# volume-em/empanada

Measured on AMD Instinct MI355X. Metric: Mvox/s end-to-end 3D panoptic inference (incl. consensus); PQ vs CPU ref, higher is better.
Workload: dtype f32

## Files before the change

empanada_amd/_hip.py:

```python
import ctypes
import os

import torch

from .tables import bits

_HERE = os.path.dirname(os.path.abspath(__file__))
LIB_PATH = os.path.join(_HERE, 'libemp_hip.so')

MAX_KS = 11
MAX_CLASSES = 16
MAX_CENTERS = 4096
CENTER_LIMIT = 65535


class HipError(RuntimeError):
    pass


_c = ctypes
_P = _c.c_void_p
_I = _c.c_int
_L = _c.c_int64
_F = _c.c_float
_U32 = _c.c_uint32

SIGNATURES = {
    'emp_version': (_I, []),
    'emp_last_error': (_c.c_char_p, []),
    'emp_device_count': (_I, []),
    'emp_bn_act_nhwc': (_I, [_P, _P, _P, _P, _I, _L, _I, _P, _L, _P]),
    'emp_dwconv_nhwc': (_I, [_P, _P, _P, _I, _I, _I, _I, _I, _P, _P]),
    'emp_upsample_bilinear': (_I, [_P, _I, _I, _I, _I, _P, _P, _I, _I, _P, _P]),
    'emp_conv_bn_act_proj_nhwc': (_I, [_P, _P, _P, _P, _I] + [_I] * 10 + [_P, _I, _P, _P, _L, _P]),
    'emp_conv_k_slab': (_I, [_L, _I, _I, _I]),
    'emp_conv_stream_eligible': (_I, [_I, _L] + [_I] * 9),
    'emp_conv_stream_walk': (_I, [_L, _I, _I, _I, _L, _P, _P]),
    'emp_conv_stream_grid': (_I, [_L, _I]),
    'emp_conv_stream_launches': (_L, []),
    'emp_conv_k_slab_cin': (_I, [_L, _I, _I, _I, _I]),
    'emp_conv_k_slab_geom': (_I, [_L, _I, _I, _I, _I, _I, _I, _I, _I]),
    'emp_conv1x1_ws_eligible': (_I, [_L, _I, _I, _I, _I, _I, _I, _I]),
    'emp_conv1x1_ws_kind_for': (_I, [_L, _I, _I, _I, _I, _I, _I, _I, _I]),
    'emp_conv1x1_ws_launches': (_L, [_I]),
    'emp_gconv_chunk': (_I, [_I]),
    'emp_gconv3x3_bn_act_nhwc': (_I, [_P, _L, _P, _P, _P, _I, _I, _I, _I, _I, _I, _I, _P, _L, _P]),
    'emp_conv_bn_act_nhwc': (_I, [_P, _P, _P, _P, _P, _L, _I] + [_I] * 10 + [_P, _L, _P]),
    'emp_conv_splitk_plan': (_I, [_L, _I, _I, _I, _I]),
    'emp_conv_splitk_bn_act_nhwc': (_I, [_P, _P, _P, _P, _P, _L, _I] + [_I] * 11 + [_P, _P, _L, _P]),
    'emp_wino_input_transform': (_I, [_P, _I, _I, _I, _I, _I, _P, _L, _P, _P]),
    'emp_gemm_nt_batched': (_I, [_P, _P, _I, _L, _I, _I, _P, _P]),
    'emp_wino4_input_transform': (_I, [_P, _I, _I, _I, _I, _I, _P, _L, _P, _P]),
    'emp_wino4_output_transform': (_I, [_P, _P, _L, _I, _I, _I, _I, _I, _P, _P, _I, _P, _L, _P]),
    'emp_wino4_conv_bn_act_nhwc': (_I, [_P, _I, _I, _I, _I, _I, _P, _L, _P, _I, _P, _P, _I, _P, _L, _P]),
    'emp_wino4_fused_eligible': (_I, [_L, _I, _I, _I]),
    'emp_wino3_input_transform': (_I, [_P, _I, _I, _I, _I, _I, _P, _L, _P, _P]),
    'emp_wino3_output_transform': (_I, [_P, _P, _L, _I, _I, _I, _I, _I, _P, _P, _I, _P, _L, _P]),
    'emp_wino_gemm_fused': (_I, [_P, _I, _I, _I, _I, _I, _P, _L, _P, _I, _P, _P]),
    'emp_wino_output_transform': (_I, [_P, _P, _L, _I, _I, _I, _I, _I, _P, _P, _I, _P, _L, _P]),
    'emp_chain_class': (_I, [_L, _P, _P, _P, _I, _P, _P, _P, _P, _L, _L, _c.c_double, _c.c_double, _P, _P, _P, _P]),
    'emp_lsap_maximize': (_L, [_P, _L, _L, _P, _P]),
    'emp_slices_to_input': (_I, [_P, _L, _L, _L, _I, _I, _I, _I, _I, _F, _F, _P, _P]),
    'emp_slices_to_input_scaled': (_I, [_P, _L, _L, _L] + [_I] * 7 + [_P, _P, _P, _P, _I, _F, _F, _P, _P]),
    'emp_pointwise_out_nhwc': (_I, [_P, _P, _P, _L, _L, _I, _I, _P, _P]),
    'emp_bn_relu_maxpool_nhwc': (_I, [_P, _P, _P, _I, _I, _I, _I, _P, _P]),
    'emp_stem_conv7_bn_relu_maxpool': (_I, [_P, _P, _P, _P, _I, _I, _I, _P, _P]),
    'emp_logits_to_prob': (_I, [_P, _I, _I, _L, _P, _P]),
    'emp_upsample_bilinear_prob': (_I, [_P, _I, _I, _I, _I, _P, _P, _I, _I, _P, _I, _P]),
    'emp_pr_upsample2x': (_I, [_P, _I, _I, _I, _I, _P, _P, _P]),
    'emp_pr_topk_work_bytes': (_L, [_I, _L]),
    'emp_pr_topk': (_I, [_P, _I, _L, _I, _P, _L, _P, _P]),
    'emp_pr_point_sample': (_I, [_P, _L, _P, _I, _I, _I, _I, _I, _P, _I, _I, _I, _P, _P, _I, _P]),
    'emp_pr_scatter': (_I, [_P, _I, _P, _I, _I, _I, _L, _P, _P]),
    'emp_median_harden_stack': (_I, [_P, _I, _I, _L, _I, _F, _P, _P, _P]),
    'emp_median_harden_window': (_I, [_P, _P, _P, _I, _I, _L, _I, _F, _P, _P, _P]),
    'emp_median_step': (_I, [_c.POINTER(_P), _I, _L, _P, _P]),
    'emp_harden': (_I, [_P, _I, _I, _L, _F, _P, _P]),
    'emp_find_centers': (_I, [_P, _I, _I, _I, _F, _I, _I, _P, _P, _P]),
    'emp_find_centers_work_elems': (_L, [_I, _I, _I, _I]),
    'emp_find_centers_ws': (_I, [_P, _I, _I, _I, _F, _I, _I, _P, _P, _P, _P]),
    'emp_group_work_elems': (_L, [_I, _I]),
    'emp_group_pixels': (_I, [_P, _P, _I, _P, _I, _I, _I, _I, _P, _U32, _P, _P, _P]),
    'emp_fuse_work_elems': (_L, [_I, _I, _I]),
    'emp_fuse_panoptic': (_I, [_P, _P, _I, _I, _I, _I, _I, _I, _U32, _L, _L, _L, _P, _P, _P, _P]),
    'emp_fuse_lut': (_I, [_P, _P, _I, _I, _I, _I, _I, _I, _U32, _L, _L, _P, _P]),
    'emp_fuse_apply': (_I, [_P, _P, _I, _I, _I, _I, _I, _I, _U32, _L, _L, _P, _P, _P, _P]),
    'emp_runs_count': (_I, [_P, _I, _I, _I, _P, _P]),
# ... 2451 lines not shown
                                               int(stride), int(pad), 2 if relu == 'gate' else int(bool(relu))))
    if Cin is not None:
        return int(load().emp_conv_k_slab_cin(int(M), int(Cout), int(batch), int(bool(has_residual)), int(Cin)))
    return int(load().emp_conv_k_slab(int(M), int(Cout), int(batch), int(bool(has_residual))))


_WINO3_G = [[0.5, 0.0, 0.0], [-0.5, -0.5, -0.5], [-1.0 / 6, 1.0 / 6, -1.0 / 6], [1.0 / 6, 1.0 / 3, 2.0 / 3], [0.0, 0.0, 1.0]]


def wino3_filter_transform(w_oihw):
    g = w_oihw.detach().double().cpu()

    def comb(a, b, c):
        return [(G[0] * a + G[1] * b) + G[2] * c for G in _WINO3_G]

    rows = comb(g[:, :, 0, :], g[:, :, 1, :], g[:, :, 2, :])
    U = []
    for r in rows:
        U.extend(comb(r[:, :, 0], r[:, :, 1], r[:, :, 2]))
    return torch.stack(U, dim=0).float().contiguous()


def wino3_conv_bn_act(x, U, tiles_dev, dil, scale=None, shift=None, relu=False, out=None):
    require_gpu()
    N, Cin, H, W = x.shape
    Cout = U.shape[1]
    assert x.is_cuda and x.dtype == torch.float32 and x.is_contiguous(memory_format=torch.channels_last)
    T = tiles_dev.shape[0]
    V = torch.empty((25, T, Cin), dtype=torch.float32, device=x.device)
    Mw = torch.empty((25, T, Cout), dtype=torch.float32, device=x.device)
    if out is None:
        out = torch.empty((N, Cout, H, W), dtype=torch.float32, device=x.device, memory_format=torch.channels_last)
    assert out.shape == (N, Cout, H, W) and out.stride(1) == 1
    ops = out.stride(3)
    assert out.stride(2) == W * ops and out.stride(0) == H * W * ops, "NHWC channel slice required"
    st = stream()
    call('emp_wino3_input_transform', x.data_ptr(), N, H, W, Cin, dil, _ptr(tiles_dev), T, _ptr(V), st,
         alg_bytes=4 * (x.numel() + V.numel()))
    call('emp_gemm_nt_batched', _ptr(V), _ptr(U), 25, T, Cout, Cin, _ptr(Mw), st,
         alg_bytes=4 * (V.numel() + U.numel() + Mw.numel()), alg_flops=2 * 25 * T * Cout * Cin)
    call('emp_wino3_output_transform', _ptr(Mw), _ptr(tiles_dev), T, N, H, W, Cout, dil, _ptr(scale), _ptr(shift),
         int(bool(relu)), out.data_ptr(), ops, st, alg_bytes=4 * (Mw.numel() + N * Cout * H * W))
    return out


def conv_bn_act_proj_nhwc(x, w_okkc, scale, shift, relu, proj_w, proj_b=None, stride=1, pad=0, dil=1, keep=False):
    require_gpu()
    N, Cin, H, W = x.shape
    Cout, KH, KW, _ = w_okkc.shape
    n = proj_w.shape[0]
    assert x.is_cuda and x.dtype == torch.float32 and x.is_contiguous(memory_format=torch.channels_last)
    OH = (H + 2 * pad - dil * (KH - 1) - 1) // stride + 1
    OW = (W + 2 * pad - dil * (KW - 1) - 1) // stride + 1
    acc = torch.zeros((N, n, OH, OW), dtype=torch.float32, device=x.device)
    act = (torch.empty((N, Cout, OH, OW), dtype=torch.float32, device=x.device, memory_format=torch.channels_last)
           if keep else None)
    call('emp_conv_bn_act_proj_nhwc', x.data_ptr(), _ptr(w_okkc), _ptr(scale), _ptr(shift), int(bool(relu)), N, H, W,
         Cin, Cout, KH, KW, stride, pad, dil, _ptr(proj_w), n, _ptr(acc), act.data_ptr() if keep else None, 0,
         stream(), alg_bytes=4 * (x.numel() + w_okkc.numel() + acc.numel() + (act.numel() if keep else 0)),
         alg_flops=2 * N * OH * OW * Cout * (Cin * KH * KW + n))
    if proj_b is not None:
        acc += proj_b.view(1, -1, 1, 1)
    return (acc, act) if keep else acc
```

empanada_amd/csrc/emp_conv.hip:

```cpp
#include "emp_common.h"
#include "emp_wino4.h"
#include <stdlib.h>

typedef float f32x16 __attribute__((ext_vector_type(16)));

#define CG_BM 128
#define CG_BK 32
#define CG_THREADS 256

struct ConvGeom {
    const float *x, *w, *scale, *shift, *res;
    float *out;
    int N, H, W, Cin, OH, OW, Cout, KH, KW, stride, pad, dil, relu;
    int64_t M, out_ps, res_ps;
    int tiles_m, tiles_n;
    int64_t x_bs, w_bs, out_bs;
    const int32_t *tiles;
    const float *proj_w;
    float *proj_out;
    int proj_n;
    int64_t hw;
};

__device__ __attribute__((aligned(16))) float cg_zero_page[64];
// ... 692 lines not shown
    const int T = g.tiles_m * g.tiles_n;
    const dim3 grid(8 * ((T + 7) / 8), 1, k_splits);
    hipStream_t st = emp_stream(stream);
    if (pl.narrow)
        hipLaunchKernelGGL((conv_igemm_f32_kernel<1, 0, false, 32, false, true>), grid, dim3(CG_THREADS), 0, st, g);
    else
        hipLaunchKernelGGL((conv_igemm_f32_kernel<2, 0, false, 32, false, true>), grid, dim3(CG_THREADS), 0, st, g);
    EMP_CHECK_LAUNCH("emp_conv_splitk_bn_act_nhwc(partials)");
    const int64_t total = g.M * (Cout / 4);
    hipLaunchKernelGGL(splitk_reduce_kernel, dim3(emp_grid(total, 256, 4096)), dim3(256), 0, st, work, k_splits, g.M, Cout,
                       scale, shift, residual, res_pixel_stride, relu, out, out_pixel_stride);
    EMP_CHECK_LAUNCH("emp_conv_splitk_bn_act_nhwc(reduce)");
    return EMP_OK;
}

extern "C" int emp_conv_bn_act_proj_nhwc(const float *x, const float *w_okkc, const float *scale, const float *shift,
                                         int relu, int N, int H, int W, int Cin, int Cout, int KH, int KW, int stride,
                                         int pad, int dil, const float *proj_w, int proj_n, float *proj_out,
                                         float *out, int64_t out_pixel_stride, void *stream)
{
    EMP_REQUIRE(x && w_okkc && proj_w && proj_out, "conv_proj: null pointer");
    EMP_REQUIRE(N >= 0 && H > 0 && W > 0 && Cin > 0 && Cin % CG_BK == 0, "conv_proj: bad shape (Cin %% %d)", CG_BK);
    EMP_REQUIRE(Cout == 128 || Cout == 256, "conv_proj: Cout %d must be 128 or 256 (at most two cout tiles)", Cout);
    EMP_REQUIRE(proj_n >= 1 && proj_n <= 4, "conv_proj: proj_n %d not in 1..4", proj_n);
    EMP_REQUIRE(KH >= 1 && KW >= 1 && KH <= 7 && KW <= 7 && stride >= 1 && dil >= 1 && pad >= 0, "conv_proj: bad filter geometry");
    const int OH = (H + 2 * pad - dil * (KH - 1) - 1) / stride + 1;
    const int OW = (W + 2 * pad - dil * (KW - 1) - 1) / stride + 1;
    EMP_REQUIRE(OH > 0 && OW > 0, "conv_proj: empty output");
    if (out_pixel_stride == 0) out_pixel_stride = Cout;
    EMP_REQUIRE(((reinterpret_cast<uintptr_t>(x) | reinterpret_cast<uintptr_t>(w_okkc) | reinterpret_cast<uintptr_t>(proj_w) |
                  reinterpret_cast<uintptr_t>(out)) & 15) == 0 && (out_pixel_stride & 3) == 0, "conv_proj: alignment");
    EMP_REQUIRE(out != x, "conv_proj: output cannot alias the input");
    if (N == 0) return EMP_OK;
    ConvGeom g;
    g.x = x; g.w = w_okkc; g.scale = scale; g.shift = shift; g.res = nullptr; g.out = out;
    g.N = N; g.H = H; g.W = W; g.Cin = Cin; g.OH = OH; g.OW = OW; g.Cout = Cout; g.KH = KH; g.KW = KW;
    g.stride = stride; g.pad = pad; g.dil = dil; g.relu = relu;
    g.M = (int64_t)N * OH * OW; g.out_ps = out_pixel_stride; g.res_ps = Cout;
    g.x_bs = g.w_bs = g.out_bs = 0; g.tiles = nullptr;
    g.proj_w = proj_w; g.proj_out = proj_out; g.proj_n = proj_n; g.hw = (int64_t)OH * OW;
    const CgPlan pl = cg_plan(g.M, Cout, 1, false, true, false);
    g.tiles_m = pl.tiles_m;
    g.tiles_n = pl.tiles_n;
    const int T = g.tiles_m * g.tiles_n;
    const int grid = 8 * ((T + 7) / 8);
#define CG_GOP(BK_, GL_) hipLaunchKernelGGL((conv_igemm_f32_kernel<2, 0, false, BK_, true, GL_>), dim3(grid), dim3(CG_THREADS), 0, emp_stream(stream), g)
    if (pl.glds) { if (pl.slab == 16) CG_GOP(16, true); else CG_GOP(32, true); }
    else { if (pl.slab == 16) CG_GOP(16, false); else CG_GOP(32, false); }
#undef CG_GOP
    EMP_CHECK_LAUNCH("emp_conv_bn_act_proj_nhwc");
    return EMP_OK;
}


__global__ __launch_bounds__(256) void wino_input_kernel(const float *__restrict__ x, const int32_t *__restrict__ tiles,
                                                         int64_t T, int H, int W, int C4, int dil, float4 *__restrict__ V)
{
    const int64_t total = T * C4;
    for (int64_t i = (int64_t)blockIdx.x * blockDim.x + threadIdx.x; i < total; i += (int64_t)gridDim.x * blockDim.x) {
        const int c4 = (int)(i % C4);
        const int64_t t = i / C4;
        const int n = tiles[3 * t], by = tiles[3 * t + 1], bx = tiles[3 * t + 2];
        const float4 *src = reinterpret_cast<const float4 *>(x) + (int64_t)n * H * W * C4 + c4;
        float4 d[4][4];
#pragma unroll
        for (int a = 0; a < 4; ++a)
#pragma unroll
            for (int b = 0; b < 4; ++b) {
                const int yy = by + a * dil, xx = bx + b * dil;
                d[a][b] = make_float4(0.f, 0.f, 0.f, 0.f);
                if (yy >= 0 && yy < H && xx >= 0 && xx < W) d[a][b] = src[((int64_t)yy * W + xx) * C4];
            }
#define W_SUB(p, q) make_float4(__fsub_rn(p.x, q.x), __fsub_rn(p.y, q.y), __fsub_rn(p.z, q.z), __fsub_rn(p.w, q.w))
#define W_ADD(p, q) make_float4(__fadd_rn(p.x, q.x), __fadd_rn(p.y, q.y), __fadd_rn(p.z, q.z), __fadd_rn(p.w, q.w))
        float4 tt[4][4];
#pragma unroll
        for (int a = 0; a < 4; ++a) {
            tt[a][0] = W_SUB(d[a][0], d[a][2]);
            tt[a][1] = W_ADD(d[a][1], d[a][2]);
            tt[a][2] = W_SUB(d[a][2], d[a][1]);
            tt[a][3] = W_SUB(d[a][1], d[a][3]);
        }
        float4 *dst = V + t * C4 + c4;
        const int64_t ps = T * C4;
#pragma unroll
        for (int v = 0; v < 4; ++v) {
            dst[(0 * 4 + v) * ps] = W_SUB(tt[0][v], tt[2][v]);
            dst[(1 * 4 + v) * ps] = W_ADD(tt[1][v], tt[2][v]);
            dst[(2 * 4 + v) * ps] = W_SUB(tt[2][v], tt[1][v]);
            dst[(3 * 4 + v) * ps] = W_SUB(tt[1][v], tt[3][v]);
        }
    }
}

__global__ __launch_bounds__(256) void wino_output_kernel(const float4 *__restrict__ Mw, const int32_t *__restrict__ tiles,
                                                          int64_t T, int H, int W, int Co4, int dil,
                                                          const float4 *__restrict__ scale, const float4 *__restrict__ shift,
                                                          int relu, float *__restrict__ out, int64_t out_ps)
{
    const int64_t total = T * Co4;
    for (int64_t i = (int64_t)blockIdx.x * blockDim.x + threadIdx.x; i < total; i += (int64_t)gridDim.x * blockDim.x) {
        const int c4 = (int)(i % Co4);
        const int64_t t = i / Co4;
        const int n = tiles[3 * t], oy = tiles[3 * t + 1] + dil, ox = tiles[3 * t + 2] + dil;
        const float4 *src = Mw + t * Co4 + c4;
        const int64_t ps = T * Co4;
// ... 387 lines not shown
```

empanada_amd/csrc/emp_conv_stream.hip:

```cpp
#include "emp_common.h"
#include <atomic>
#include <stdlib.h>
#include <type_traits>

typedef float f32x16 __attribute__((ext_vector_type(16)));

#define CS_BM 128
#define CS_BN 128
#define CS_BK 16
#define CS_THREADS 256
#define CS_RING 3
#define CS_RESIDENT 768

struct StreamGeom {
    const float *x, *w, *scale, *shift;
    float *out;
    int Cin, Cout, tiles_n;
    int64_t M, out_ps;
    int64_t tiles, total;
    int64_t x_bs, w_bs, out_bs;
};

__host__ __device__ static inline int64_t cs_walk(int64_t total, int grid, int b, int64_t step)
{
    const int64_t chunk = (total + 7) >> 3;
    const int64_t local = (b >> 3) + step * (grid >> 3);
    if (local >= chunk) return -1;
    const int64_t u = (b & 7) * chunk + local;
    return u < total ? u : -1;
}
__host__ __device__ static inline int64_t cs_walk_steps(int64_t total, int grid, int b)
{
    const int64_t chunk = (total + 7) >> 3;
    int64_t end = total - (b & 7) * chunk;
    if (end > chunk) end = chunk;
    const int64_t first = b >> 3, stride = grid >> 3;
    return end > first ? (end - first + stride - 1) / stride : 0;
}

extern "C" int emp_conv_stream_walk(int64_t tiles, int batch, int grid, int block, int64_t step, int64_t *entry, int64_t *tile)
{
    if (tiles <= 0 || batch <= 0 || grid <= 0 || (grid & 7) || block < 0 || block >= grid || step < 0) return 0;
    const int64_t u = cs_walk(tiles * batch, grid, block, step);
    if (u < 0 || step >= cs_walk_steps(tiles * batch, grid, block)) return 0;
    if (entry) *entry = u / tiles;
    if (tile) *tile = u % tiles;
    return 1;
}

static inline int cs_grid(int64_t total)
{
    const int64_t g = 8 * ((total + 7) / 8);
    return (int)(g < CS_RESIDENT ? g : CS_RESIDENT);
}
extern "C" int emp_conv_stream_grid(int64_t tiles, int batch) { return tiles > 0 && batch > 0 ? cs_grid(tiles * batch) : 0; }

__device__ __forceinline__ void cs_glds16(const float *base, unsigned lane_off, unsigned lds_byte_addr)
{
    asm volatile("s_mov_b32 m0, %2\n\ts_nop 4\n\tglobal_load_lds_dwordx4 %0, %1" ::"v"(lane_off), "s"(base), "s"(lds_byte_addr) : "memory", "m0");
}
__device__ __forceinline__ void cs_store2(float *dst, float v0, float v1)
{
    asm volatile("global_store_dword %0, %1, off\n\tglobal_store_dword %0, %2, off offset:128" ::"v"(dst), "v"(v0), "v"(v1) : "memory");
}
template <int N>
__device__ __forceinline__ void cs_wait_vm()
{
    asm volatile("s_waitcnt vmcnt(%0)" ::"n"(N) : "memory");
}

template <bool AFFINE, bool RELU>
__global__ __launch_bounds__(CS_THREADS, 3) void conv_stream_f32_kernel(StreamGeom g)
{
    constexpr int BK = CS_BK, TPR = BK / 4, RPP = CS_THREADS / TPR, AR = CS_BM / RPP, BROWS = CS_BN / RPP;
    constexpr int NF4 = BK / 8, RPW = 64 / TPR, NL = AR + BROWS;
    constexpr int A_ELEMS = CS_RING * CS_BM * BK, B_ELEMS = CS_RING * CS_BN * BK;
    __shared__ __attribute__((aligned(16))) float smem[A_ELEMS + B_ELEMS];
    float *As = smem, *Bs = smem + A_ELEMS;

    const int b = blockIdx.x, grid = gridDim.x;
    const int nt = (int)cs_walk_steps(g.total, grid, b);
    if (nt == 0) return;
    const int S = g.Cin / BK;
    const int n_slabs = nt * S;
    const int64_t u0 = cs_walk(g.total, grid, b, 0);
    const int64_t ustep = grid >> 3;

    const int tid = threadIdx.x;
    const int lrow = tid / TPR;
    const int wave = tid >> 6, lane = tid & 63;
    const int wm = wave >> 1, wn = wave & 1;
    const int r = lane & 31, hh = lane >> 5;
    const int csw = (((tid % TPR) ^ ((lrow >> 2) & 3)) * 4);
    const int swz_rd = (r >> 2) & 3;

    auto locate = [&](int64_t u, int64_t &entry, int64_t &m0, int &n0) {
        const unsigned uu = (unsigned)u, tiles = (unsigned)g.tiles, tn_ = (unsigned)g.tiles_n;
        const unsigned e = g.total == g.tiles ? 0u : uu / tiles;
        const unsigned t = uu - e * tiles;
        const unsigned tm = t / tn_;
        entry = e;
        m0 = (int64_t)tm * CS_BM;
        n0 = (int)(t - tm * tn_) * CS_BN;
    };

    const float *a_base = nullptr, *b_base = nullptr;
    unsigned voff_a[AR];
    const unsigned voff_b = (unsigned)(lrow * g.Cin + csw) * 4u;
    int ld_k = 0, ld_c0 = 0, ld_ring = 0;
    auto set_ld_tile = [&](int k) {
        int64_t entry, m0;
        int n0;
        locate(u0 + k * ustep, entry, m0, n0);
        a_base = g.x + entry * g.x_bs + m0 * g.Cin;
        b_base = g.w + entry * g.w_bs + (int64_t)n0 * g.Cin;
        const int last = (int)(g.M - m0 < CS_BM ? g.M - m0 : CS_BM) - 1;
#pragma unroll
        for (int i = 0; i < AR; ++i) {
            const int row = lrow + RPP * i;
            voff_a[i] = (unsigned)((row < last ? row : last) * g.Cin + csw) * 4u;
        }
    };
    const unsigned lds0 = (unsigned)(size_t)(__attribute__((address_space(3))) float *)smem;
    const unsigned a_dst = __builtin_amdgcn_readfirstlane(lds0 + (unsigned)(RPW * wave * BK * 4));
    const unsigned b_dst = __builtin_amdgcn_readfirstlane(lds0 + (unsigned)((A_ELEMS + RPW * wave * BK) * 4));
    auto issue_slab = [&]() {
#pragma unroll
        for (int i = 0; i < AR; ++i)
            cs_glds16(a_base + ld_c0, voff_a[i], a_dst + (unsigned)((ld_ring * CS_BM + RPP * i) * BK * 4));
#pragma unroll
        for (int i = 0; i < BROWS; ++i)
            cs_glds16(b_base + (int64_t)(RPP * i) * g.Cin + ld_c0, voff_b, b_dst + (unsigned)((ld_ring * CS_BN + RPP * i) * BK * 4));
        ld_ring = ld_ring == CS_RING - 1 ? 0 : ld_ring + 1;
        ld_c0 += BK;
        if (ld_c0 == g.Cin) {
            ld_c0 = 0;
            ++ld_k;
            if (ld_k < nt) set_ld_tile(ld_k);
        }
    };

    int cp_k = 0, cp_s = 0, rd_ring = 0;
    int sc_n0 = -1;
    float sc[2] = {1.f, 1.f}, sh[2] = {0.f, 0.f};
    auto load_affine = [&](int n0) {
        if constexpr (AFFINE) {
#pragma unroll
            for (int j = 0; j < 2; ++j) {
                sc[j] = g.scale[n0 + wn * 64 + j * 32 + r];
                sh[j] = g.shift[n0 + wn * 64 + j * 32 + r];
            }
            asm volatile("" : "+v"(sc[0]), "+v"(sc[1]), "+v"(sh[0]), "+v"(sh[1]));
        }
        sc_n0 = n0;
    };

    f32x16 acc[2][2];
#pragma unroll
    for (int i = 0; i < 2; ++i)
#pragma unroll
        for (int j = 0; j < 2; ++j)
#pragma unroll
            for (int q = 0; q < 16; ++q) acc[i][j][q] = 0.f;

    auto epilogue = [&](int k) {
        int64_t entry, m0;
        int n0;
        locate(u0 + k * ustep, entry, m0, n0);
        if (n0 != sc_n0) load_affine(n0);
        float *obase = g.out + entry * g.out_bs + (m0 + wm * 64 + 4 * hh) * g.out_ps + n0 + wn * 64 + r;
        const bool whole = m0 + CS_BM <= g.M;
        auto rows = [&](auto checked) {
#pragma unroll
            for (int i = 0; i < 2; ++i)
#pragma unroll
                for (int q = 0; q < 16; ++q) {
                    const int row = i * 32 + (q & 3) + 8 * (q >> 2);
                    float v[2];
#pragma unroll
                    for (int j = 0; j < 2; ++j) {
                        v[j] = acc[i][j][q];
                        if constexpr (AFFINE) v[j] = __fadd_rn(__fmul_rn(v[j], sc[j]), sh[j]);
                        if constexpr (RELU) v[j] = fmaxf(v[j], 0.f);
                    }
                    if (!decltype(checked)::value || m0 + wm * 64 + 4 * hh + row < g.M) cs_store2(obase + row * g.out_ps, v[0], v[1]);
                }
        };
        if (whole) rows(std::false_type{}); else rows(std::true_type{});
#pragma unroll
        for (int i = 0; i < 2; ++i)
#pragma unroll
            for (int j = 0; j < 2; ++j)
#pragma unroll
                for (int q = 0; q < 16; ++q) acc[i][j][q] = 0.f;
    };

    {
        int64_t entry, m0;
        int n0;
        locate(u0, entry, m0, n0);
        load_affine(n0);
    }
    set_ld_tile(0);

    issue_slab();
    if (n_slabs > 1) issue_slab();
    if (n_slabs > 1) cs_wait_vm<NL>(); else cs_wait_vm<0>();
    __builtin_amdgcn_s_barrier();
    for (int s = 0; s < n_slabs; ++s) {
        const bool more = s + 2 < n_slabs;
        if (more) issue_slab();
        const float *Ar = &As[rd_ring * CS_BM * BK + (wm * 64 + r) * BK];
        const float *Br = &Bs[rd_ring * CS_BN * BK + (wn * 64 + r) * BK];
#pragma unroll
        for (int f = 0; f < NF4; ++f) {
            const int pc = (((hh * NF4 + f) ^ swz_rd) * 4);
            float4 fa[2], fb[2];
#pragma unroll
            for (int i = 0; i < 2; ++i) fa[i] = *reinterpret_cast<const float4 *>(Ar + i * 32 * BK + pc);
#pragma unroll
            for (int j = 0; j < 2; ++j) fb[j] = *reinterpret_cast<const float4 *>(Br + j * 32 * BK + pc);
#pragma unroll
            for (int e = 0; e < 4; ++e) {
                float av[2], bv[2];
#pragma unroll
                for (int i = 0; i < 2; ++i) av[i] = e == 0 ? fa[i].x : e == 1 ? fa[i].y : e == 2 ? fa[i].z : fa[i].w;
#pragma unroll
                for (int j = 0; j < 2; ++j) bv[j] = e == 0 ? fb[j].x : e == 1 ? fb[j].y : e == 2 ? fb[j].z : fb[j].w;
#pragma unroll
                for (int i = 0; i < 2; ++i)
#pragma unroll
                    for (int j = 0; j < 2; ++j)
                        acc[i][j] = __builtin_amdgcn_mfma_f32_32x32x2f32(av[i], bv[j], acc[i][j], 0, 0, 0);
            }
        }
        rd_ring = rd_ring == CS_RING - 1 ? 0 : rd_ring + 1;
        if (more) cs_wait_vm<NL>(); else cs_wait_vm<0>();
        __builtin_amdgcn_s_barrier();
        if (++cp_s == S) {
            epilogue(cp_k);
            cp_s = 0;
            ++cp_k;
        }
    }
}

static std::atomic<int64_t> cs_launches;
extern "C" int64_t emp_conv_stream_launches(void) { return cs_launches.load(); }

extern "C" __attribute__((visibility("hidden"))) int emp_conv_stream_launch(const float *x, const float *w, const float *scale, const float *shift,
                                                                            int relu, int batch, int64_t M, int Cin, int Cout,
                                                                            int64_t x_bs, int64_t w_bs, int64_t out_bs, float *out,
                                                                            int64_t out_ps, void *stream)
{
    EMP_REQUIRE(x && w && out && (scale != nullptr) == (shift != nullptr), "conv_stream: null pointer");
    EMP_REQUIRE(batch >= 1 && M > 0 && Cin > 0 && Cin % CS_BK == 0 && Cout > 0 && Cout % CS_BN == 0, "conv_stream: bad shape");
    EMP_REQUIRE(scale || !relu, "conv_stream: ReLU needs scale and shift");
    StreamGeom g;
    g.x = x; g.w = w; g.scale = scale; g.shift = shift; g.out = out;
    g.Cin = Cin; g.Cout = Cout; g.tiles_n = Cout / CS_BN;
    g.M = M; g.out_ps = out_ps;
    g.tiles = emp_cdiv(M, CS_BM) * g.tiles_n;
    g.total = g.tiles * batch;
    g.x_bs = x_bs; g.w_bs = w_bs; g.out_bs = out_bs;
    const int grid = cs_grid(g.total);
    EMP_REQUIRE(g.total < (1LL << 28) && (g.total / grid + 2) * (Cin / CS_BK) < (1LL << 30), "conv_stream: too many tiles");
    hipStream_t st = emp_stream(stream);
    if (!scale) hipLaunchKernelGGL((conv_stream_f32_kernel<false, false>), dim3(grid), dim3(CS_THREADS), 0, st, g);
    else if (relu) hipLaunchKernelGGL((conv_stream_f32_kernel<true, true>), dim3(grid), dim3(CS_THREADS), 0, st, g);
    else hipLaunchKernelGGL((conv_stream_f32_kernel<true, false>), dim3(grid), dim3(CS_THREADS), 0, st, g);
    EMP_CHECK_LAUNCH("emp_conv_stream_launch");
    ++cs_launches;
    return EMP_OK;
}
```

include/emp_hip.h:

```cpp
#ifndef EMP_HIP_H
#define EMP_HIP_H

#include <stdint.h>

#ifdef __cplusplus
extern "C" {
#endif

#define EMP_OK 0
#define EMP_EINVAL (-1)
#define EMP_ELAUNCH (-2)
#define EMP_ENODEV (-3)

#define EMP_MAX_KS 11
#define EMP_MAX_CLASSES 16
#define EMP_MAX_CENTERS 4096
#define EMP_CENTER_LIMIT 65535

int emp_version(void);
const char *emp_last_error(void);
int emp_device_count(void);

int emp_slices_to_input(const uint8_t *vol, int64_t stride_slice, int64_t stride_row, int64_t stride_col,
                        int n_slices, int h, int w, int hp, int wp, float mean255, float inv_std255,
                        float *out, void *stream);

int emp_slices_to_input_scaled(const uint8_t *vol, int64_t stride_slice, int64_t stride_row, int64_t stride_col,
                               int n_slices, int h, int w, int dh, int dw, int hp, int wp, const int32_t *row_off,
                               const int16_t *row_coef, const int32_t *col_off, const int16_t *col_coef, int area,
                               float mean255, float inv_std255, float *out, void *stream);

int emp_bn_act_nhwc(const float *x, const float *scale, const float *shift, const float *residual,
                    int relu, int64_t n_pixels, int C, float *out, int64_t out_pixel_stride, void *stream);

int emp_dwconv_nhwc(const float *x, const float *w_kkc, const float *bias, int N, int H, int W, int C,
                    int k, float *y, void *stream);

int emp_upsample_bilinear(const float *x, int N, int C, int h, int w, const int64_t *x_strides,
                          float *y, int H, int W, const int64_t *y_strides, void *stream);

int emp_conv_k_slab(int64_t M, int Cout, int batch, int has_residual);
int emp_conv_k_slab_cin(int64_t M, int Cout, int batch, int has_residual, int Cin);
int emp_conv_k_slab_geom(int64_t M, int Cout, int has_residual, int Cin, int KH, int KW, int stride, int pad, int relu);
int emp_conv1x1_ws_eligible(int64_t M, int Cin, int Cout, int KH, int KW, int stride, int pad, int relu);
int emp_conv1x1_ws_kind_for(int64_t M, int Cin, int Cout, int KH, int KW, int stride, int pad, int relu, int has_residual);
int64_t emp_conv1x1_ws_launches(int kind);
int emp_conv_stream_eligible(int batch, int64_t M, int Cin, int Cout, int KH, int KW, int stride, int pad, int relu,
                             int has_residual, int proj);
int emp_conv_stream_grid(int64_t tiles, int batch);
int emp_conv_stream_walk(int64_t tiles, int batch, int grid, int block, int64_t step, int64_t *entry, int64_t *tile);
int64_t emp_conv_stream_launches(void);
int emp_conv_bn_act_nhwc(const float *x, const float *w_okkc, const float *scale, const float *shift,
                         const float *residual, int64_t res_pixel_stride, int relu, int N, int H, int W,
                         int Cin, int Cout, int KH, int KW, int stride, int pad, int dil, float *out,
                         int64_t out_pixel_stride, void *stream);
int emp_conv_splitk_plan(int64_t M, int Cout, int Cin, int KH, int KW);
int emp_conv_splitk_bn_act_nhwc(const float *x, const float *w_okkc, const float *scale, const float *shift,
                                const float *residual, int64_t res_pixel_stride, int relu, int N, int H, int W,
                                int Cin, int Cout, int KH, int KW, int stride, int pad, int dil, int k_splits,
                                float *work, float *out, int64_t out_pixel_stride, void *stream);

int emp_conv_bn_act_proj_nhwc(const float *x, const float *w_okkc, const float *scale, const float *shift,
                              int relu, int N, int H, int W, int Cin, int Cout, int KH, int KW, int stride,
                              int pad, int dil, const float *proj_w, int proj_n, float *proj_out,
                              float *out, int64_t out_pixel_stride, void *stream);

int emp_gconv_chunk(int group_w);
int emp_gconv3x3_bn_act_nhwc(const float *x, int64_t x_pixel_stride, const float *w_okkc, const float *scale,
                             const float *shift, int relu, int N, int H, int W, int groups, int group_w,
                             int stride, float *out, int64_t out_pixel_stride, void *stream);

int emp_wino_input_transform(const float *x, int N, int H, int W, int C, int dil, const int32_t *tiles,
                             int64_t T, float *V, void *stream);
int emp_gemm_nt_batched(const float *A, const float *B, int batch, int64_t M, int N, int K, float *C,
                        void *stream);
int emp_wino_gemm_fused(const float *x, int N, int H, int W, int Cin, int dil, const int32_t *tiles,
                        int64_t T, const float *U, int Cout, float *Mw, void *stream);
int emp_wino_output_transform(const float *Mw, const int32_t *tiles, int64_t T, int N, int H, int W,
                              int Cout, int dil, const float *scale, const float *shift, int relu,
                              float *out, int64_t out_pixel_stride, void *stream);

int emp_wino4_input_transform(const float *x, int N, int H, int W, int C, int dil, const int32_t *tiles,
                              int64_t T, float *V, void *stream);
int emp_wino4_output_transform(const float *Mw, const int32_t *tiles, int64_t T, int N, int H, int W,
                               int Cout, int dil, const float *scale, const float *shift, int relu,
                               float *out, int64_t out_pixel_stride, void *stream);
int emp_wino4_conv_bn_act_nhwc(const float *x, int N, int H, int W, int Cin, int dil, const int32_t *tiles, int64_t T,
                               const float *U, int Cout, const float *scale, const float *shift, int relu,
                               float *out, int64_t out_pixel_stride, void *stream);
int emp_wino4_fused_eligible(int64_t T, int Cin, int Cout, int has_scale_shift);

int emp_wino3_input_transform(const float *x, int N, int H, int W, int C, int dil, const int32_t *tiles,
                              int64_t T, float *V, void *stream);
int emp_wino3_output_transform(const float *Mw, const int32_t *tiles, int64_t T, int N, int H, int W,
                               int Cout, int dil, const float *scale, const float *shift, int relu,
                               float *out, int64_t out_pixel_stride, void *stream);

int emp_pointwise_out_nhwc(const float *x, const float *w, const float *bias, int64_t n_pixels,
                           int64_t pixels_per_image, int C, int Cout, float *out, void *stream);

int emp_bn_relu_maxpool_nhwc(const float *x, const float *scale, const float *shift, int N, int H, int W,
                             int C, float *y, void *stream);

int emp_stem_conv7_bn_relu_maxpool(const float *x, const float *w_tc, const float *scale, const float *shift,
                                   int N, int H, int W, float *y, void *stream);

int emp_logits_to_prob(const float *logits, int N, int C, int64_t HW, float *prob, void *stream);

int emp_upsample_bilinear_prob(const float *x, int N, int C, int h, int w, const int64_t *x_strides,
                               float *y, int H, int W, const int64_t *y_strides, int prob, void *stream);

int emp_median_harden_stack(const float *prob, int D, int C, int64_t HW, int ks, float thr,
                            uint8_t *out_sem, float *out_prob, void *stream);

int emp_median_harden_window(const float *hist, const float *prob, const float *halo, int D, int C, int64_t HW,
                             int ks, float thr, uint8_t *out_sem, float *out_tail, void *stream);

int emp_median_step(const float *const *slices_host, int ks, int64_t n, float *out, void *stream);
// ... 259 lines not shown
```

Measured before the change: 137.7.

## Fuse 1x1 conv+BN+ReLU with projection head into persistent streaming kernel

Adds a PROJ variant of the persistent streaming conv kernel that computes the 1x1 conv, applies BN+ReLU, and reduces against the small projection weights in the epilogue. It uses DPP quad shuffles plus an LDS chain reduction and carries partial sums across the two Cout tiles, so the projection output is written directly with its bias instead of using atomics into a zeroed buffer. The torch zero-fill and separate bias add are removed from the Python path, and the fallback uses dedicated zero and bias kernels. The price is a more complex epilogue with extra barriers and LDS staging, and it only applies to eligible 1x1 shapes with Cout of 128 or 256.

```diff
diff --git a/empanada_amd/_hip.py b/empanada_amd/_hip.py
--- a/empanada_amd/_hip.py
+++ b/empanada_amd/_hip.py
@@ -33,6 +33,10 @@
     'emp_dwconv_nhwc': (_I, [_P, _P, _P, _I, _I, _I, _I, _I, _P, _P]),
     'emp_upsample_bilinear': (_I, [_P, _I, _I, _I, _I, _P, _P, _I, _I, _P, _P]),
     'emp_conv_bn_act_proj_nhwc': (_I, [_P, _P, _P, _P, _I] + [_I] * 10 + [_P, _I, _P, _P, _L, _P]),
+    'emp_conv_bn_act_proj_bias_nhwc': (_I, [_P, _P, _P, _P, _I] + [_I] * 10 + [_P, _P, _I, _P, _P, _L, _P]),
+    'emp_conv_stream_proj_eligible': (_I, [_L] + [_I] * 8),
+    'emp_conv_stream_proj_launches': (_L, []),
+    'emp_conv_stream_proj_walk': (_I, [_L, _I, _I, _I, _L, _P, _P]),
     'emp_conv_k_slab': (_I, [_L, _I, _I, _I]),
     'emp_conv_stream_eligible': (_I, [_I, _L] + [_I] * 9),
     'emp_conv_stream_walk': (_I, [_L, _I, _I, _I, _L, _P, _P]),
@@ -2590,13 +2594,15 @@
     assert x.is_cuda and x.dtype == torch.float32 and x.is_contiguous(memory_format=torch.channels_last)
     OH = (H + 2 * pad - dil * (KH - 1) - 1) // stride + 1
     OW = (W + 2 * pad - dil * (KW - 1) - 1) // stride + 1
-    acc = torch.zeros((N, n, OH, OW), dtype=torch.float32, device=x.device)
+    acc = torch.empty((N, n, OH, OW), dtype=torch.float32, device=x.device)
     act = (torch.empty((N, Cout, OH, OW), dtype=torch.float32, device=x.device, memory_format=torch.channels_last)
            if keep else None)
-    call('emp_conv_bn_act_proj_nhwc', x.data_ptr(), _ptr(w_okkc), _ptr(scale), _ptr(shift), int(bool(relu)), N, H, W,
-         Cin, Cout, KH, KW, stride, pad, dil, _ptr(proj_w), n, _ptr(acc), act.data_ptr() if keep else None, 0,
-         stream(), alg_bytes=4 * (x.numel() + w_okkc.numel() + acc.numel() + (act.numel() if keep else 0)),
+    if proj_b is not None:
+        _expect('conv_bn_act_proj_nhwc: proj_b', proj_b, torch.float32, numel=n)
+        assert proj_b.is_contiguous()
+    call('emp_conv_bn_act_proj_bias_nhwc', x.data_ptr(), _ptr(w_okkc), _ptr(scale), _ptr(shift), int(bool(relu)), N, H, W,
+         Cin, Cout, KH, KW, stride, pad, dil, _ptr(proj_w), _ptr(proj_b), n, _ptr(acc),
+         act.data_ptr() if keep else None, 0, stream(), profile_as='emp_conv_bn_act_proj_nhwc',
+         alg_bytes=4 * (x.numel() + w_okkc.numel() + acc.numel() + (act.numel() if keep else 0)),
          alg_flops=2 * N * OH * OW * Cout * (Cin * KH * KW + n))
-    if proj_b is not None:
-        acc += proj_b.view(1, -1, 1, 1)
     return (acc, act) if keep else acc
diff --git a/empanada_amd/csrc/emp_conv.hip b/empanada_amd/csrc/emp_conv.hip
--- a/empanada_amd/csrc/emp_conv.hip
+++ b/empanada_amd/csrc/emp_conv.hip
@@ -768,6 +768,52 @@
     return EMP_OK;
 }
 
+extern "C" __attribute__((visibility("hidden"))) int emp_conv_stream_proj_launch(const float *x, const float *w, const float *scale, const float *shift,
+                                                                                 int64_t M, int64_t hw, int Cin, int Cout, const float *proj_w,
+                                                                                 const float *proj_bias, int proj_n, float *proj_out, float *out,
+                                                                                 int64_t out_ps, void *stream);
+extern "C" __attribute__((visibility("hidden"))) int emp_conv_proj_zero_launch(float *acc, int64_t total, void *stream);
+extern "C" __attribute__((visibility("hidden"))) int emp_conv_proj_bias_launch(float *acc, const float *bias, int64_t N, int n, int64_t hw, void *stream);
+
+extern "C" int emp_conv_stream_proj_eligible(int64_t M, int Cin, int Cout, int KH, int KW, int stride, int pad, int relu, int proj_n)
+{
+    static const char *off = getenv("EMP_CONV_NO_STREAM");
+    const char *mint = getenv("EMP_CONV_STREAM_MIN_TILES");
+    if (off && off[0] == '1') return 0;
+    if (M <= 0 || M >= (1LL << 31) || Cin <= 0 || Cin % CG_BK != 0 || (Cout != 128 && Cout != 256)) return 0;
+    if (!(KH == 1 && KW == 1 && stride == 1 && pad == 0 && relu == 1) || proj_n < 1 || proj_n > 4) return 0;
+    const CgPlan pl = cg_plan(M, Cout, 1, false, true, false);
+    if (!(pl.slab == 16 && pl.glds && !pl.narrow)) return 0;
+    const int64_t total = (int64_t)pl.tiles_m * pl.tiles_n;
+    if (mint) return pl.tiles_m >= atoll(mint) * emp_conv_stream_grid(pl.tiles_m, 1);
+    return total >= CS_MIN_TOTAL;
+}
+
+extern "C" int emp_conv_bn_act_proj_bias_nhwc(const float *x, const float *w_okkc, const float *scale, const float *shift,
+                                              int relu, int N, int H, int W, int Cin, int Cout, int KH, int KW, int stride,
+                                              int pad, int dil, const float *proj_w, const float *proj_bias, int proj_n,
+                                              float *proj_out, float *out, int64_t out_pixel_stride, void *stream)
+{
+    EMP_REQUIRE(x && w_okkc && proj_w && proj_out, "conv_proj_bias: null pointer");
+    EMP_REQUIRE(N >= 0 && H > 0 && W > 0 && Cin > 0 && Cout > 0 && KH >= 1 && KW >= 1 && stride >= 1 && dil >= 1 && pad >= 0 &&
+                proj_n >= 1 && proj_n <= 4, "conv_proj_bias: bad shape");
+    if (N == 0) return EMP_OK;
+    const int64_t OH = (H + 2 * pad - dil * (KH - 1) - 1) / stride + 1, OW = (W + 2 * pad - dil * (KW - 1) - 1) / stride + 1;
+    const int64_t ops = out_pixel_stride ? out_pixel_stride : Cout;
+    const bool aligned = ((reinterpret_cast<uintptr_t>(x) | reinterpret_cast<uintptr_t>(w_okkc) | reinterpret_cast<uintptr_t>(out)) & 15) == 0 &&
+                         (ops & 3) == 0 && ops >= Cout && out != x;
+    if (aligned && scale && shift && OH > 0 && OW > 0 &&
+        emp_conv_stream_proj_eligible(N * OH * OW, Cin, Cout, KH, KW, stride, pad, relu, proj_n))
+        return emp_conv_stream_proj_launch(x, w_okkc, scale, shift, N * OH * OW, OH * OW, Cin, Cout, proj_w, proj_bias, proj_n,
+                                           proj_out, out, ops, stream);
+    int rc = OH > 0 && OW > 0 ? emp_conv_proj_zero_launch(proj_out, N * proj_n * OH * OW, stream) : EMP_OK;
+    if (rc != EMP_OK) return rc;
+    rc = emp_conv_bn_act_proj_nhwc(x, w_okkc, scale, shift, relu, N, H, W, Cin, Cout, KH, KW, stride, pad, dil, proj_w,
+                                             proj_n, proj_out, out, out_pixel_stride, stream);
+    if (rc != EMP_OK || !proj_bias) return rc;
+    return emp_conv_proj_bias_launch(proj_out, proj_bias, N, proj_n, OH * OW, stream);
+}
+
 
 __global__ __launch_bounds__(256) void wino_input_kernel(const float *__restrict__ x, const int32_t *__restrict__ tiles,
                                                          int64_t T, int H, int W, int C4, int dil, float4 *__restrict__ V)
diff --git a/empanada_amd/csrc/emp_conv_stream.hip b/empanada_amd/csrc/emp_conv_stream.hip
--- a/empanada_amd/csrc/emp_conv_stream.hip
+++ b/empanada_amd/csrc/emp_conv_stream.hip
@@ -20,6 +20,12 @@
     int64_t tiles, total;
     int64_t x_bs, w_bs, out_bs;
 };
+struct StreamProjGeom : StreamGeom {
+    const float *proj_w, *proj_bias;
+    float *proj_out;
+    int proj_n;
+    unsigned hw;
+};
 
 __host__ __device__ static inline int64_t cs_walk(int64_t total, int grid, int b, int64_t step)
 {
@@ -68,19 +74,32 @@
 {
     asm volatile("s_waitcnt vmcnt(%0)" ::"n"(N) : "memory");
 }
-
-template <bool AFFINE, bool RELU>
-__global__ __launch_bounds__(CS_THREADS, 3) void conv_stream_f32_kernel(StreamGeom g)
-{
+__device__ __forceinline__ void cs_lds_barrier()
+{
+    asm volatile("s_waitcnt lgkmcnt(0)\n\ts_barrier" ::: "memory");
+}
+template <int E>
+__device__ __forceinline__ float cs_quad(float x)
+{
+    return __int_as_float(__builtin_amdgcn_mov_dpp(__float_as_int(x), E * 0x55, 0xf, 0xf, false));
+}
+
+template <bool AFFINE, bool RELU, bool PROJ = false>
+__global__ __launch_bounds__(CS_THREADS, 3) void conv_stream_f32_kernel(std::conditional_t<PROJ, StreamProjGeom, StreamGeom> g)
+{
+    static_assert(!PROJ || (AFFINE && RELU), "the PROJ form is built for BN + ReLU");
     constexpr int BK = CS_BK, TPR = BK / 4, RPP = CS_THREADS / TPR, AR = CS_BM / RPP, BROWS = CS_BN / RPP;
     constexpr int NF4 = BK / 8, RPW = 64 / TPR, NL = AR + BROWS;
     constexpr int A_ELEMS = CS_RING * CS_BM * BK, B_ELEMS = CS_RING * CS_BN * BK;
-    __shared__ __attribute__((aligned(16))) float smem[A_ELEMS + B_ELEMS];
+    constexpr int W_LD = 256, W_ELEMS = PROJ ? 4 * W_LD : 0;
+    __shared__ __attribute__((aligned(16))) float smem[A_ELEMS + B_ELEMS + W_ELEMS];
     float *As = smem, *Bs = smem + A_ELEMS;
 
     const int b = blockIdx.x, grid = gridDim.x;
-    const int nt = (int)cs_walk_steps(g.total, grid, b);
-    if (nt == 0) return;
+    const int nu = (int)cs_walk_steps(g.total, grid, b);
+    if (nu == 0) return;
+    int nt = nu;
+    if constexpr (PROJ) nt = nu * g.tiles_n;
     const int S = g.Cin / BK;
     const int n_slabs = nt * S;
     const int64_t u0 = cs_walk(g.total, grid, b, 0);
@@ -103,6 +122,15 @@
         m0 = (int64_t)tm * CS_BM;
         n0 = (int)(t - tm * tn_) * CS_BN;
     };
+    auto locate_k = [&](int k, int64_t &entry, int64_t &m0, int &n0) {
+        if constexpr (PROJ) {
+            const int tsh = g.tiles_n - 1;
+            entry = 0;
+            m0 = (u0 + (k >> tsh) * ustep) * CS_BM;
+            n0 = (k & tsh) * CS_BN;
+        } else
+            locate(u0 + k * ustep, entry, m0, n0);
+    };
 
     const float *a_base = nullptr, *b_base = nullptr;
     unsigned voff_a[AR];
@@ -111,7 +139,7 @@
     auto set_ld_tile = [&](int k) {
         int64_t entry, m0;
         int n0;
-        locate(u0 + k * ustep, entry, m0, n0);
+        locate_k(k, entry, m0, n0);
         a_base = g.x + entry * g.x_bs + m0 * g.Cin;
         b_base = g.w + entry * g.w_bs + (int64_t)n0 * g.Cin;
         const int last = (int)(g.M - m0 < CS_BM ? g.M - m0 : CS_BM) - 1;
@@ -195,7 +223,133 @@
                 for (int q = 0; q < 16; ++q) acc[i][j][q] = 0.f;
     };
 
-    {
+    float *Ws = smem + A_ELEMS + B_ELEMS;
+    float scp[2][2] = {{1.f, 1.f}, {1.f, 1.f}}, shp[2][2] = {{0.f, 0.f}, {0.f, 0.f}};
+    float pbias = 0.f, carry0 = 0.f, carry1 = 0.f;
+    int pn = 1, lg = 2;
+    if constexpr (PROJ) {
+        pn = g.proj_n;
+        lg = pn == 1 ? 2 : pn == 2 ? 1 : 0;
+    }
+    const int rpr_lg = 5 + lg;
+    auto epilogue_proj = [&](int k) {
+        if constexpr (PROJ) {
+            int64_t entry, m0;
+            int n0;
+            locate_k(k, entry, m0, n0);
+            const int tn = n0 / CS_BN;
+            float scj[2], shj[2];
+#pragma unroll
+            for (int j = 0; j < 2; ++j) {
+                scj[j] = tn ? scp[1][j] : scp[0][j];
+                shj[j] = tn ? shp[1][j] : shp[0][j];
+            }
+            const int fs = rd_ring == 0 ? CS_RING - 1 : rd_ring - 1;
+            float *stage = smem + fs * (CS_BM * BK);
+            auto chain_at = [&](int ch) { return stage + (ch >> 6) * A_ELEMS + (ch & 63) * 32; };
+            const float *wl = Ws + n0 + wn * 64 + r;
+            if (g.out) {
+                int64_t ops = g.out_ps;
+                asm volatile("" : "+s"(ops));
+                float *obase = g.out + (m0 + wm * 64 + 4 * hh) * ops + n0 + wn * 64 + r;
+                const int lim = (int)(g.M - m0 < CS_BM ? g.M - m0 : CS_BM) - (wm * 64 + 4 * hh);
+#pragma unroll
+                for (int i = 0; i < 2; ++i)
+#pragma unroll
+                    for (int q = 0; q < 16; ++q) {
+                        const int row = i * 32 + (q & 3) + 8 * (q >> 2);
+                        const float v0 = fmaxf(__fadd_rn(__fmul_rn(acc[i][0][q], scj[0]), shj[0]), 0.f);
+                        const float v1 = fmaxf(__fadd_rn(__fmul_rn(acc[i][1][q], scj[1]), shj[1]), 0.f);
+                        if (row < lim) cs_store2(obase + row * ops, v0, v1);
+                    }
+            }
+            const int pass0 = __builtin_amdgcn_readfirstlane(wm * 2);
+            const int c0 = wn * 16 + (r >> 2);
+            int wo[4];
+#pragma unroll
+            for (int s = 0; s < 4; ++s) wo[s] = ((((c0 >> 2) ^ (4 * hh)) ^ s) << 2) + (c0 & 3);
+            for (int rd = 0; rd < (4 >> lg); ++rd) {
+                if (rd > 0) cs_lds_barrier();
+#pragma unroll
+                for (int i = 0; i < 2; ++i) {
+                    const int pass = pass0 + i;
+                    if ((pass >> lg) != rd) continue;
+                    const int rl0 = ((pass & ((1 << lg) - 1)) << 5) + 4 * hh;
+#pragma unroll 1
+                    for (int qq = 0; qq < pn; ++qq) {
+                        const float w0 = wl[qq * W_LD], w1 = wl[qq * W_LD + 32];
+                        float *cb = chain_at((qq << rpr_lg) + rl0);
+#pragma unroll
+                        for (int q = 0; q < 16; ++q) {
+                            const int row = (q & 3) + 8 * (q >> 2);
+                            const float v0 = fmaxf(__fadd_rn(__fmul_rn(acc[i][0][q], scj[0]), shj[0]), 0.f);
+                            const float v1 = fmaxf(__fadd_rn(__fmul_rn(acc[i][1][q], scj[1]), shj[1]), 0.f);
+                            const float x0 = __fmul_rn(v0, w0), x1 = __fmul_rn(v1, w1);
+                            const float p0 = __fadd_rn(__fadd_rn(__fadd_rn(x0, cs_quad<1>(x0)), cs_quad<2>(x0)), cs_quad<3>(x0));
+                            const float p1 = __fadd_rn(__fadd_rn(__fadd_rn(x1, cs_quad<1>(x1)), cs_quad<2>(x1)), cs_quad<3>(x1));
+                            if ((r & 3) == 0) {
+                                cb[row * 32 + wo[q & 3]] = p0;
+                                cb[row * 32 + wo[(q & 3) ^ 2]] = p1;
+                            }
+                        }
+                    }
+                }
+                cs_lds_barrier();
+                const int ch = tid & 127;
+                if ((tid >> 7) == (rd & 1) && ch < (pn << rpr_lg)) {
+                    const float *cb = chain_at(ch);
+                    float t = 0.f;
+#pragma unroll
+                    for (int c4 = 0; c4 < 8; ++c4) {
+                        const float4 p4 = *reinterpret_cast<const float4 *>(cb + ((c4 ^ (ch & 7)) << 2));
+                        t = c4 == 0 ? p4.x : __fadd_rn(t, p4.x);
+                        t = __fadd_rn(__fadd_rn(__fadd_rn(t, p4.y), p4.z), p4.w);
+                    }
+                    if (g.tiles_n == 2 && tn == 0) {
+                        if (rd >> 1) carry1 = t; else carry0 = t;
+                    } else {
+                        float res = __fadd_rn(0.f, g.tiles_n == 2 ? (rd >> 1 ? carry1 : carry0) : t);
+                        if (g.tiles_n == 2) res = __fadd_rn(res, t);
+                        if (g.proj_bias) res = __fadd_rn(res, pbias);
+                        const int qq = ch >> rpr_lg;
+                        const int64_t p = m0 + (rd << rpr_lg) + (ch & ((1 << rpr_lg) - 1));
+                        if (p < g.M) {
+                            const unsigned pu = (unsigned)p, img = pu / g.hw;
+                            g.proj_out[((int64_t)img * pn + qq) * g.hw + (pu - img * g.hw)] = res;
+                        }
+                    }
+                }
+            }
+            cs_lds_barrier();
+#pragma unroll
+            for (int i = 0; i < 2; ++i)
+#pragma unroll
+                for (int j = 0; j < 2; ++j)
+#pragma unroll
+                    for (int q = 0; q < 16; ++q) acc[i][j][q] = 0.f;
+        }
+    };
+
+    if constexpr (PROJ) {
+        for (int idx = tid; idx < pn * g.Cout; idx += CS_THREADS) {
+            const int q = idx / g.Cout;
+            Ws[q * W_LD + idx - q * g.Cout] = g.proj_w[idx];
+        }
+#pragma unroll
+        for (int t = 0; t < 2; ++t)
+            if (t < g.tiles_n) {
+#pragma unroll
+                for (int j = 0; j < 2; ++j) {
+                    scp[t][j] = g.scale[t * CS_BN + wn * 64 + j * 32 + r];
+                    shp[t][j] = g.shift[t * CS_BN + wn * 64 + j * 32 + r];
+                }
+            }
+        const int myq = (tid & 127) >> rpr_lg;
+        if (g.proj_bias && myq < pn) pbias = g.proj_bias[myq];
+        asm volatile("" : "+v"(scp[0][0]), "+v"(scp[0][1]), "+v"(scp[1][0]), "+v"(scp[1][1]), "+v"(shp[0][0]), "+v"(shp[0][1]),
+                          "+v"(shp[1][0]), "+v"(shp[1][1]), "+v"(pbias));
+        asm volatile("s_waitcnt vmcnt(0) lgkmcnt(0)" ::: "memory");
+    } else {
         int64_t entry, m0;
         int n0;
         locate(u0, entry, m0, n0);
@@ -238,7 +392,7 @@
         if (more) cs_wait_vm<NL>(); else cs_wait_vm<0>();
         __builtin_amdgcn_s_barrier();
         if (++cp_s == S) {
-            epilogue(cp_k);
+            if constexpr (PROJ) epilogue_proj(cp_k); else epilogue(cp_k);
             cp_s = 0;
             ++cp_k;
         }
@@ -273,3 +427,66 @@
     ++cs_launches;
     return EMP_OK;
 }
+
+static std::atomic<int64_t> cs_proj_launches;
+extern "C" int64_t emp_conv_stream_proj_launches(void) { return cs_proj_launches.load(); }
+
+extern "C" __attribute__((visibility("hidden"))) int emp_conv_stream_proj_launch(const float *x, const float *w, const float *scale, const float *shift,
+                                                                                 int64_t M, int64_t hw, int Cin, int Cout, const float *proj_w,
+                                                                                 const float *proj_bias, int proj_n, float *proj_out, float *out,
+                                                                                 int64_t out_ps, void *stream)
+{
+    EMP_REQUIRE(x && w && scale && shift && proj_w && proj_out, "conv_stream_proj: null pointer");
+    EMP_REQUIRE(M > 0 && M < (1LL << 31) && hw > 0 && hw <= M && Cin > 0 && Cin % CS_BK == 0 && (Cout == CS_BN || Cout == 2 * CS_BN),
+                "conv_stream_proj: bad shape");
+    EMP_REQUIRE(proj_n >= 1 && proj_n <= 4, "conv_stream_proj: proj_n %d not in 1..4", proj_n);
+    StreamProjGeom g;
+    g.x = x; g.w = w; g.scale = scale; g.shift = shift; g.out = out;
+    g.Cin = Cin; g.Cout = Cout; g.tiles_n = Cout / CS_BN;
+    g.M = M; g.out_ps = out_ps;
+    g.tiles = g.total = emp_cdiv(M, CS_BM);
+    g.x_bs = g.w_bs = g.out_bs = 0;
+    g.proj_w = proj_w; g.proj_bias = proj_bias; g.proj_out = proj_out; g.proj_n = proj_n; g.hw = (unsigned)hw;
+    const int grid = cs_grid(g.total);
+    EMP_REQUIRE((g.total / grid + 2) * g.tiles_n * (Cin / CS_BK) < (1LL << 30), "conv_stream_proj: too many tiles");
+    hipLaunchKernelGGL((conv_stream_f32_kernel<true, true, true>), dim3(grid), dim3(CS_THREADS), 0, emp_stream(stream), g);
+    EMP_CHECK_LAUNCH("emp_conv_stream_proj_launch");
+    ++cs_proj_launches;
+    return EMP_OK;
+}
+
+__global__ __launch_bounds__(256) void conv_proj_zero_kernel(float *__restrict__ acc, int64_t total)
+{
+    for (int64_t i = (int64_t)blockIdx.x * blockDim.x + threadIdx.x; i < total; i += (int64_t)gridDim.x * blockDim.x) acc[i] = 0.f;
+}
+extern "C" __attribute__((visibility("hidden"))) int emp_conv_proj_zero_launch(float *acc, int64_t total, void *stream)
+{
+    if (total <= 0) return EMP_OK;
+    hipLaunchKernelGGL(conv_proj_zero_kernel, dim3(emp_grid(total, 256, 4096)), dim3(256), 0, emp_stream(stream), acc, total);
+    EMP_CHECK_LAUNCH("emp_conv_proj_zero_launch");
+    return EMP_OK;
+}
+__global__ __launch_bounds__(256) void conv_proj_bias_kernel(float *__restrict__ acc, const float *__restrict__ bias, int n, int64_t hw, int64_t total)
+{
+    for (int64_t i = (int64_t)blockIdx.x * blockDim.x + threadIdx.x; i < total; i += (int64_t)gridDim.x * blockDim.x)
+        acc[i] = __fadd_rn(acc[i], bias[(i / hw) % n]);
+}
+extern "C" __attribute__((visibility("hidden"))) int emp_conv_proj_bias_launch(float *acc, const float *bias, int64_t N, int n, int64_t hw, void *stream)
+{
+    const int64_t total = N * n * hw;
+    if (total <= 0) return EMP_OK;
+    hipLaunchKernelGGL(conv_proj_bias_kernel, dim3(emp_grid(total, 256, 4096)), dim3(256), 0, emp_stream(stream), acc, bias, n, hw, total);
+    EMP_CHECK_LAUNCH("emp_conv_proj_bias_launch");
+    return EMP_OK;
+}
+
+extern "C" int emp_conv_stream_proj_walk(int64_t units, int cout_tiles, int grid, int block, int64_t k, int64_t *unit, int *cout_tile)
+{
+    if (units <= 0 || (cout_tiles != 1 && cout_tiles != 2) || grid <= 0 || (grid & 7) || block < 0 || block >= grid || k < 0) return 0;
+    const int tsh = cout_tiles - 1;
+    if ((k >> tsh) >= cs_walk_steps(units, grid, block)) return 0;
+    const int64_t u = cs_walk(units, grid, block, 0) + (k >> tsh) * (grid >> 3);
+    if (unit) *unit = u;
+    if (cout_tile) *cout_tile = (int)(k & tsh);
+    return 1;
+}
diff --git a/include/emp_hip.h b/include/emp_hip.h
--- a/include/emp_hip.h
+++ b/include/emp_hip.h
@@ -64,6 +64,15 @@
                               int relu, int N, int H, int W, int Cin, int Cout, int KH, int KW, int stride,
                               int pad, int dil, const float *proj_w, int proj_n, float *proj_out,
                               float *out, int64_t out_pixel_stride, void *stream);
+int emp_conv_bn_act_proj_bias_nhwc(const float *x, const float *w_okkc, const float *scale, const float *shift,
+                                   int relu, int N, int H, int W, int Cin, int Cout, int KH, int KW, int stride,
+                                   int pad, int dil, const float *proj_w, const float *proj_bias, int proj_n,
+                                   float *proj_out, float *out, int64_t out_pixel_stride, void *stream);
+int emp_conv_stream_proj_eligible(int64_t M, int Cin, int Cout, int KH, int KW, int stride, int pad, int relu,
+                                  int proj_n);
+int64_t emp_conv_stream_proj_launches(void);
+int emp_conv_stream_proj_walk(int64_t units, int cout_tiles, int grid, int block, int64_t k, int64_t *unit,
+                              int *cout_tile);
 
 int emp_gconv_chunk(int group_w);
 int emp_gconv3x3_bn_act_nhwc(const float *x, int64_t x_pixel_stride, const float *w_okkc, const float *scale,
```

Result: faster. 139.2, median of 6 (+1.0%).
